# imalexlee/simple-vk-renderer

Hardware: AMD Instinct MI355X
Metric: shaded fragments/s (higher is better)
Workload: dtype f32

## Files before the change

simple-vk-renderer_amd/csrc/k_tile.hip:

```cpp
#include <hip/hip_ext.h>

#include <cstdlib>
#include <type_traits>

#include "svr_launch.h"
#include "svr_pixel.h"
#include "svr_span.h"

namespace svr {

constexpr uint32_t REC_COMMON = 0x80000000u;
#ifndef SVR_PRIO_COST
#define SVR_PRIO_COST 200u
#endif
constexpr int BATCH = 64;
constexpr uint32_t SREC = 7;

constexpr float kG0 = 0x1.c51282p-2f, kG1 = -0x1.14a3a2p-2f, kG2 = 0x1.37536ap-3f, kG3 = -0x1.778474p-5f;

__device__ __forceinline__ float lod_from_rho2(float rho2) {
  uint32_t bits = f2u(rho2);
  int e = (int)(bits >> 23) - 127;
  float m = u2f((bits & 0x7fffffu) | 0x3f800000u);
  float t = m - 1.0f;
  float g = fmaf(fmaf(fmaf(kG3, t, kG2), t, kG1), t, kG0);
  float s = t * (1.0f - t);
  float l = fmaf(s, g, t);
  float lam = 0.5f * ((float)e + l);
  lam = (rho2 <= 0x1p+100f) ? lam : 50.0f;
  lam = (rho2 >= 0x1p-100f) ? lam : -50.0f;
  return lam;
}

__device__ __forceinline__ float lerpf(float a, float b, float t) { return fmaf(t, b - a, a); }
__device__ __forceinline__ float clamp_med3(float x, float lo, float hi) { return __builtin_amdgcn_fmed3f(x, lo, hi); }
__device__ __forceinline__ double top_left_bias(uint32_t flags, uint32_t bit) { return (double)((flags / bit) & 1u); }

struct TexD {
  uint32_t base_off;
  uint32_t w, h, lw, lh, levels, filters;
  float min_lod, max_lod;
};

struct Taps {
  uint32_t o00, o10, o01, o11;
  float alpha, beta;
};
__device__ __forceinline__ Taps level_taps(int wl, int hl, uint32_t plw, uint32_t base, bool linear, float u, float v) {
  float U = (u - floorf(u)) * (float)wl;
  float V = (v - floorf(v)) * (float)hl;
  float Uh = U - 0.5f, Vh = V - 0.5f;
  float fu = floorf(linear ? Uh : U), fv = floorf(linear ? Vh : V);
  Taps tp;
  tp.alpha = linear ? Uh - fu : 0.0f;
  tp.beta = linear ? Vh - fv : 0.0f;
  int i0 = (int)fu, j0 = (int)fv;
  int i1 = linear ? i0 + 1 : i0, j1 = linear ? j0 + 1 : j0;
  if (i0 < 0) i0 += wl;
  if (i0 >= wl) i0 -= wl;
  if (i1 >= wl) i1 -= wl;
  if (j0 < 0) j0 += hl;
  if (j0 >= hl) j0 -= hl;
  if (j1 >= hl) j1 -= hl;
  const uint32_t x0 = texel_offset_x((uint32_t)i0), x1 = texel_offset_x((uint32_t)i1);
  const uint32_t y0 = base + texel_offset_y(plw, (uint32_t)j0), y1 = base + texel_offset_y(plw, (uint32_t)j1);
  tp.o00 = y0 + x0;
  tp.o10 = y0 + x1;
  tp.o01 = y1 + x0;
  tp.o11 = y1 + x1;
  return tp;
}
__device__ __forceinline__ Taps level_taps_exp(int kw, int kh, uint32_t plw, uint32_t base, float u, float v) {
  float U = ldexpf(u - floorf(u), kw);
  float V = ldexpf(v - floorf(v), kh);
  float Uh = U - 0.5f, Vh = V - 0.5f;
  float fu = floorf(Uh), fv = floorf(Vh);
  Taps tp;
  tp.alpha = Uh - fu;
  tp.beta = Vh - fv;
  const int i0 = (int)fu, j0 = (int)fv;
  const uint32_t mw = (1u << kw) - 1u, mh = (1u << kh) - 1u;
  const uint32_t x0 = texel_offset_x((uint32_t)i0 & mw), x1 = texel_offset_x((uint32_t)(i0 + 1) & mw);
  const uint32_t y0 = base + texel_offset_y(plw, (uint32_t)j0 & mh), y1 = base + texel_offset_y(plw, (uint32_t)(j0 + 1) & mh);
  tp.o00 = y0 + x0;
  tp.o10 = y0 + x1;
  tp.o01 = y1 + x0;
  tp.o11 = y1 + x1;
  return tp;
}
__device__ __forceinline__ uint32_t texel(const uint8_t* arena, uint32_t off) {
  return *reinterpret_cast<const uint32_t*>(arena + off);
}
__device__ __forceinline__ float bilerp(uint32_t t00, uint32_t t10, uint32_t t01, uint32_t t11, int c, float a, float b) {
  return lerpf(lerpf(chan(t00, c), chan(t10, c), a), lerpf(chan(t01, c), chan(t11, c), a), b);
}

__device__ __forceinline__ float4 common_texture(const uint8_t* tb, uint32_t base_off, uint32_t tk, uint32_t info, int dhi, int dlo,
                                                 float delta, float u, float v) {
  const uint32_t lw = info & 0xffu, lh = (info >> 8) & 0xffu;
  auto kexp = [](uint32_t l, int d) { return (int)__builtin_elementwise_sub_sat(l, (uint32_t)d); };
  const uint32_t bhi = base_off + packed_mip_offset(tk, (uint32_t)dhi);
  const Taps th = level_taps_exp(kexp(lw, dhi), kexp(lh, dhi), packed_level_lw(info, (uint32_t)dhi), bhi, u, v);
  const uint32_t h00 = texel(tb, th.o00), h10 = texel(tb, th.o10), h01 = texel(tb, th.o01), h11 = texel(tb, th.o11);
  float4 tx;
  tx.w = 1.0f;
  const bool two_levels = __any(delta != 0.0f);
  Taps tl = th;
  uint32_t l00 = 0, l10 = 0, l01 = 0, l11 = 0;
  if (two_levels) {
    const uint32_t blo = dlo != dhi ? bhi + packed_level_bytes(tk, (uint32_t)dhi) : bhi;
    tl = level_taps_exp(kexp(lw, dlo), kexp(lh, dlo), packed_level_lw(info, (uint32_t)dlo), blo, u, v);
    l00 = texel(tb, tl.o00), l10 = texel(tb, tl.o10), l01 = texel(tb, tl.o01), l11 = texel(tb, tl.o11);
  }
  tx.x = bilerp(h00, h10, h01, h11, 0, th.alpha, th.beta);
  tx.y = bilerp(h00, h10, h01, h11, 1, th.alpha, th.beta);
  tx.z = bilerp(h00, h10, h01, h11, 2, th.alpha, th.beta);
  if (two_levels) {
    tx.x = lerpf(tx.x, bilerp(l00, l10, l01, l11, 0, tl.alpha, tl.beta), delta);
    tx.y = lerpf(tx.y, bilerp(l00, l10, l01, l11, 1, tl.alpha, tl.beta), delta);
    tx.z = lerpf(tx.z, bilerp(l00, l10, l01, l11, 2, tl.alpha, tl.beta), delta);
  }
  return tx;
}

__device__ __forceinline__ float interp3(float a0, float da1, float da2, float b1, float b2, float r) {
  return fmaf(b2, da2, fmaf(b1, da1, a0)) * r;
}

struct FragAttr {
  float b1, b2, r, u, v, nx, ny, nz, light, cr, cg, cb, won;
};

__device__ __forceinline__ float quad_partner_x(float v) { return u2f((uint32_t)__builtin_amdgcn_mov_dpp((int)f2u(v), 0xB1, 0xf, 0xf, true)); }
__device__ __forceinline__ float quad_partner_y(float v) { return u2f((uint32_t)__builtin_amdgcn_mov_dpp((int)f2u(v), 0x128, 0xf, 0xf, true)); }
template <bool TRACE, bool COMMON = false, bool ATTR = false>
__device__ __forceinline__ float4 shade_pixel(const FrameParams& P, uint32_t rec, int px, int py, float* trace, const bool quads = false,
                                              FragAttr* fa = nullptr) {
  const TriRec* tr = P.recs + rec;
  const uint4* q4 = reinterpret_cast<const uint4*>(tr);
  const float4* f4 = reinterpret_cast<const float4*>(tr);
  const double2* d2 = reinterpret_cast<const double2*>(tr);
  uint4 hdr = q4[0];
  float4 zrow = f4[1];
  double2 c2 = d2[2], c3 = d2[3], c4 = d2[4], c5 = d2[5], c6 = d2[6];
  uint4 td = q4[7];
  float4 s0 = f4[8], s1 = f4[9], s2 = f4[10], s3 = f4[11], s4 = f4[12], s5 = f4[13], s6 = f4[14];
  uint32_t flags = hdr.w;
  float inv_area = zrow.w;
  double A1, B1, A2, B2, e1, e2;
  double C1 = c5.y, C2 = c6.x;
  A1 = c2.y; B1 = c4.x; A2 = c3.x; B2 = c4.y;
  double dx = (double)px, dy = (double)py;
  e1 = fma(A1, dx, fma(B1, dy, C1)) + top_left_bias(flags, F_T1);
  e2 = fma(A2, dx, fma(B2, dy, C2)) + top_left_bias(flags, F_T2);
  TexD t;
  t.base_off = (uint32_t)(unsigned long long)__double_as_longlong(c6.y);
  const uint32_t tk = (uint32_t)((unsigned long long)__double_as_longlong(c6.y) >> 32);
  t.w = td.x & 0xffffu;
  t.h = td.x >> 16;
  t.lw = td.y & 0xffu;
  t.lh = (td.y >> 8) & 0xffu;
  t.levels = (td.y >> 16) & 0xffu;
  t.filters = td.y >> 24;
  t.min_lod = u2f(td.z);
  t.max_lod = u2f(td.w);
  float b1 = (float)e1 * inv_area, b2 = (float)e2 * inv_area;
  float q0 = s0.x, dq1 = s0.y, dq2 = s0.z;
  const float qq = fmaf(b2, dq2, fmaf(b1, dq1, q0));
  float hb1 = 0.0f, hb2 = 0.0f, vb1 = 0.0f, vb2 = 0.0f, hq = 1.0f, vq = 1.0f, hr = 0.0f, vr = 0.0f;
  auto partners = [&]() {
    if (COMMON) {
      const int sx = (int)((uint32_t)px << 31), sy = (int)((uint32_t)py << 31);
      auto flip = [](double a, int s) { return __hiloint2double(__double2hiint(a) ^ s, __double2loint(a)); };
      hb1 = (float)(e1 + flip(A1, sx)) * inv_area, hb2 = (float)(e2 + flip(A2, sx)) * inv_area;
      vb1 = (float)(e1 + flip(B1, sy)) * inv_area, vb2 = (float)(e2 + flip(B2, sy)) * inv_area;
    } else {
      double sxp = (px & 1) ? -1.0 : 1.0, syp = (py & 1) ? -1.0 : 1.0;
      hb1 = (float)fma(sxp, A1, e1) * inv_area, hb2 = (float)fma(sxp, A2, e2) * inv_area;
      vb1 = (float)fma(syp, B1, e1) * inv_area, vb2 = (float)fma(syp, B2, e2) * inv_area;
    }
    hq = fmaf(hb2, dq2, fmaf(hb1, dq1, q0)), vq = fmaf(vb2, dq2, fmaf(vb1, dq1, q0));
  };
  if (!COMMON && !quads) partners();
  const float r = COMMON ? rcp_in_window(qq) : rcp_ieee(qq);
  const uint32_t kind = COMMON ? (uint32_t)PIPE_MESH : ((flags >> F_KIND_SHIFT) & 3u);
  float cr = interp3(s1.z, s3.z, s5.z, b1, b2, r);
  float cg = interp3(s1.w, s3.w, s5.w, b1, b2, r);
  float cb = interp3(s2.x, s4.x, s6.x, b1, b2, r);
  if (ATTR) { fa->b1 = b1; fa->b2 = b2; fa->r = r; fa->won = 1.0f; }
  if (kind == PIPE_COLORED_TRIANGLE) return make_float4(cr, cg, cb, 1.0f);
  float u = interp3(s2.y, s4.y, s6.y, b1, b2, r), v = interp3(s2.z, s4.z, s6.z, b1, b2, r);
  if (ATTR) { fa->u = u; fa->v = v; }
  if (!COMMON) {
    hr = rcp_ieee(hq);
    vr = rcp_ieee(vq);
  }
  float uh, vh, uv_, vv_;
  if (quads) {
    uh = quad_partner_x(u), vh = quad_partner_x(v);
    uv_ = quad_partner_y(u), vv_ = quad_partner_y(v);
  } else {
    if (COMMON) {
      partners();
      hr = rcp_in_window(hq);
      vr = rcp_in_window(vq);
    }
    uh = interp3(s2.y, s4.y, s6.y, hb1, hb2, hr), vh = interp3(s2.z, s4.z, s6.z, hb1, hb2, hr);
    uv_ = interp3(s2.y, s4.y, s6.y, vb1, vb2, vr), vv_ = interp3(s2.z, s4.z, s6.z, vb1, vb2, vr);
  }
  float dudx = (COMMON || !(px & 1)) ? (uh - u) : (u - uh);
  float dvdx = (COMMON || !(px & 1)) ? (vh - v) : (v - vh);
  float dudy = (COMMON || !(py & 1)) ? (uv_ - u) : (u - uv_);
  float dvdy = (COMMON || !(py & 1)) ? (vv_ - v) : (v - vv_);
  float W0 = (float)t.w, H0 = (float)t.h;
  float mx = COMMON ? ldexpf(dudx, (int)t.lw) : dudx * W0, my = COMMON ? ldexpf(dvdx, (int)t.lh) : dvdx * H0;
  float nx_ = COMMON ? ldexpf(dudy, (int)t.lw) : dudy * W0, ny_ = COMMON ? ldexpf(dvdy, (int)t.lh) : dvdy * H0;
  float rho2 = fmaxf(fmaf(mx, mx, my * my), fmaf(nx_, nx_, ny_ * ny_));
  float lambda = COMMON ? clamp_med3(lod_from_rho2(rho2), t.min_lod, t.max_lod) : fminf(fmaxf(lod_from_rho2(rho2), t.min_lod), t.max_lod);
  const bool linear = COMMON ? true : (((lambda <= 0.0f) ? (t.filters & 1u) : ((t.filters >> 1) & 1u)) != 0u);
  int q = COMMON ? (int)(tk >> 24) : (int)t.levels - 1;
  const bool mip_linear = COMMON ? true : (((t.filters >> 2) & 1u) != 0u);
  int dn = min(max((int)ceilf(lambda + 0.5f) - 1, 0), q);
  float lc = COMMON ? clamp_med3(lambda, 0.0f, (float)q) : fminf(fmaxf(lambda, 0.0f), (float)q);
  float fl = floorf(lc);
  int dhi = mip_linear ? (int)fl : dn;
  float delta = mip_linear ? lc - fl : 0.0f;
  int dlo = mip_linear ? min(dhi + 1, q) : dn;
  float us = (COMMON || fabsf(u) < 8388608.0f) ? u : 0.0f, vs = (COMMON || fabsf(v) < 8388608.0f) ? v : 0.0f;
  float4 tx;
  if constexpr (COMMON) {
    tx = common_texture(P.tex_arena, t.base_off, tk, td.y, dhi, dlo, delta, us, vs);
  } else {
    const int whi = (int)max(t.w >> dhi, 1u), hhi = (int)max(t.h >> dhi, 1u);
    const uint32_t bhi = t.base_off + mip_offset(t.lw, t.lh, (uint32_t)dhi);
    const uint32_t plw_hi = level_lw(t.lw, (uint32_t)dhi);
    Taps th = level_taps(whi, hhi, plw_hi, bhi, linear, us, vs);
    const uint8_t* tb = P.tex_arena;
    uint32_t h00 = texel(tb, th.o00), h10 = texel(tb, th.o10), h01 = texel(tb, th.o01), h11 = texel(tb, th.o11);
    const bool two_levels = __any(delta != 0.0f);
    Taps tl = th;
    uint32_t l00 = 0, l10 = 0, l01 = 0, l11 = 0;
    if (two_levels) {
      const int wlo = (int)max(t.w >> dlo, 1u), hlo = (int)max(t.h >> dlo, 1u);
      const uint32_t step = level_bytes(t.lw, t.lh, (uint32_t)dhi);
      const uint32_t blo = dlo != dhi ? bhi + step : bhi;
      const uint32_t plw_lo = level_lw(t.lw, (uint32_t)dlo);
      tl = level_taps(wlo, hlo, plw_lo, blo, linear, us, vs);
      l00 = texel(tb, tl.o00);
      l10 = texel(tb, tl.o10);
      l01 = texel(tb, tl.o01);
      l11 = texel(tb, tl.o11);
    }
    tx.x = bilerp(h00, h10, h01, h11, 0, th.alpha, th.beta);
    tx.y = bilerp(h00, h10, h01, h11, 1, th.alpha, th.beta);
    tx.z = bilerp(h00, h10, h01, h11, 2, th.alpha, th.beta);
    tx.w = 1.0f;
    if (two_levels) {
      tx.x = lerpf(tx.x, bilerp(l00, l10, l01, l11, 0, tl.alpha, tl.beta), delta);
      tx.y = lerpf(tx.y, bilerp(l00, l10, l01, l11, 1, tl.alpha, tl.beta), delta);
      tx.z = lerpf(tx.z, bilerp(l00, l10, l01, l11, 2, tl.alpha, tl.beta), delta);
    }
    if (TRACE) {
      trace[0] = (float)(hdr.z >> 2); trace[1] = b1; trace[2] = b2; trace[3] = r; trace[4] = u; trace[5] = v;
      trace[6] = dudx; trace[7] = dvdx; trace[8] = dudy; trace[9] = dvdy; trace[10] = lambda;
      trace[11] = tx.x; trace[12] = tx.y; trace[13] = tx.z;
      trace[26] = hb1; trace[27] = hb2; trace[28] = vb1; trace[29] = vb2; trace[30] = hr; trace[31] = vr;
    }
    if (kind == PIPE_TEX_IMAGE) {
      tx.w = bilerp(h00, h10, h01, h11, 3, th.alpha, th.beta);
      if (two_levels) tx.w = lerpf(tx.w, bilerp(l00, l10, l01, l11, 3, tl.alpha, tl.beta), delta);
      return tx;
    }
  }
  float nx = interp3(s0.w, s2.w, s4.w, b1, b2, r);
  float ny = interp3(s1.x, s3.x, s5.x, b1, b2, r);
  float nz = interp3(s1.y, s3.y, s5.y, b1, b2, r);
  const float* L = P.scene.sunlight_direction;
  float d = fmaf(nz, L[2], fmaf(ny, L[1], nx * L[0]));
  float light = fmaxf(d, 0.1f);
  float sunw = P.scene.sunlight_color[3];
  cr = cr * tx.x;
  cg = cg * tx.y;
  cb = cb * tx.z;
  float4 o;
  o.x = fmaf(cr * light, sunw, cr * P.scene.ambient_color[0]);
  o.y = fmaf(cg * light, sunw, cg * P.scene.ambient_color[1]);
  o.z = fmaf(cb * light, sunw, cb * P.scene.ambient_color[2]);
  o.w = 1.0f;
  if (TRACE) {
    trace[15] = nx; trace[16] = ny; trace[17] = nz; trace[18] = cr; trace[19] = cg; trace[20] = cb;
    trace[21] = light; trace[22] = o.x; trace[23] = o.y; trace[24] = o.z; trace[25] = o.w;
  }
  if (ATTR) { fa->nx = nx; fa->ny = ny; fa->nz = nz; fa->light = light; fa->cr = cr; fa->cg = cg; fa->cb = cb; }
  return o;
}

template <bool INSTR, bool LIST, bool HIZ>
__device__ __forceinline__ void scan_columns(const FrameParams& P, uint4* s_cov, const uint32_t* s_list, uint32_t bin_base, uint32_t n,
                                             unsigned long long* s_depth, uint32_t* s_bm, int tx0, int ty0, int ry0, int nrows,
                                             uint32_t& n_raster, uint32_t& n_hiz_bad, uint32_t& occl) {
  auto entry = [&](uint32_t i) -> uint32_t { return LIST ? (s_list[i] & 0x7fffffffu) : P.bins[bin_base + i]; };
  const uint32_t lane = threadIdx.x & 63u, wave = threadIdx.x >> 6;
  static_assert(BATCH * 8 == 512, "two pieces per thread");
  uint4 pre0 = make_uint4(0, 0, 0, 0), pre1 = pre0;
  {
    uint32_t cnt = min((uint32_t)BATCH, n);
    const bool staged = (threadIdx.x & 7u) < SREC;
    if (staged && threadIdx.x < cnt * 8u) pre0 = reinterpret_cast<const uint4*>(P.recs + entry(threadIdx.x >> 3))[threadIdx.x & 7u];
    if (staged && threadIdx.x + 256u < cnt * 8u) pre1 = reinterpret_cast<const uint4*>(P.recs + entry(32u + (threadIdx.x >> 3)))[threadIdx.x & 7u];
  }
  constexpr uint32_t SVR_HIZ_MIN = BATCH;
  constexpr uint32_t SVR_HIZ_KEEP_COLS = 192u;
  const bool hiz = HIZ && n > (uint32_t)SVR_HIZ_MIN;
  uint32_t cur = 0, hz_cols = 0, hz_batches = 0, hz_pause = 0;
  if (hiz && threadIdx.x < 32u) s_bm[threadIdx.x] = threadIdx.x < 16u ? 0u : 0xffffffffu;
  for (uint32_t b0 = 0; b0 < n; b0 += BATCH) {
    uint32_t cnt = min((uint32_t)BATCH, n - b0);
    __syncthreads();
    const bool test = hiz && b0 && hz_pause == 0u;
    if (hiz && b0 && hz_pause) hz_pause--;
    if (test) {
      cur ^= 1u;
      const uint32_t b = threadIdx.x >> 4, k = threadIdx.x & 15u;
      const uint4* c4 = reinterpret_cast<const uint4*>(s_depth + ((b & 3u) * 8u + (k >> 1)) * TILE + (b >> 2) * 8u + (k & 1u) * 4u);
      const uint4 lo = c4[0], hi = c4[1];
      atomicMin(&s_bm[cur * 16u + b], min(min(lo.y, lo.w), min(hi.y, hi.w)));
      if (threadIdx.x < 16u) s_bm[(cur ^ 1u) * 16u + threadIdx.x] = 0xffffffffu;
    }
    if (threadIdx.x < cnt * 8u && (threadIdx.x & 7u) < SREC) s_cov[(threadIdx.x >> 3) * SREC + (threadIdx.x & 7u)] = pre0;
    if (threadIdx.x + 256u < cnt * 8u && (threadIdx.x & 7u) < SREC) s_cov[(32u + (threadIdx.x >> 3)) * SREC + (threadIdx.x & 7u)] = pre1;
    __syncthreads();
    const uint4* bm4 = reinterpret_cast<const uint4*>(s_bm + cur * 16u);
    if (b0 + BATCH < n) {
      uint32_t nb = b0 + BATCH, ncnt = min((uint32_t)BATCH, n - nb);
      const bool staged = (threadIdx.x & 7u) < SREC;
      if (staged && threadIdx.x < ncnt * 8u) pre0 = reinterpret_cast<const uint4*>(P.recs + entry(nb + (threadIdx.x >> 3)))[threadIdx.x & 7u];
      if (staged && threadIdx.x + 256u < ncnt * 8u) pre1 = reinterpret_cast<const uint4*>(P.recs + entry(nb + 32u + (threadIdx.x >> 3)))[threadIdx.x & 7u];
    }
    int cx0 = 0, cw = 0;
    bool hidden = false;
    uint32_t gone = 0;
    uint32_t zb = 0, claim = 0;
    if (lane < cnt) {
      uint4 h = s_cov[lane * SREC];
      int minx = (int)(int16_t)(h.x & 0xffffu), miny = (int)(int16_t)(h.x >> 16);
      int maxx = (int)(int16_t)(h.y & 0xffffu), maxy = (int)(int16_t)(h.y >> 16);
      cx0 = max(minx, tx0);
      const int cx1 = min(maxx, tx0 + TILE - 1);
      const int cy0 = max(miny, ry0), cy1 = min(maxy, ry0 + nrows - 1);
      cw = (cx1 >= cx0 && cy1 >= cy0) ? cx1 - cx0 + 1 : 0;
      if (HIZ && cw) {
        const float4 zr = reinterpret_cast<const float4*>(s_cov)[lane * SREC + 1u];
        const float eps = (fabsf(zr.x) + fabsf(zr.y) + fabsf(zr.z)) * 0x1p-21f;
        zb = f2u(fmaxf(fmaxf(zr.x, fmaxf(zr.x + zr.y, zr.x + zr.z)) + eps, 0.0f));
        if (minx <= tx0 && maxx >= tx0 + TILE - 1 && miny <= ry0 && maxy >= ry0 + nrows - 1) {
          const double* dd = reinterpret_cast<const double*>(s_cov + lane * SREC);
          const float x0 = (float)tx0, x1 = (float)(tx0 + TILE - 1), y0 = (float)ry0, y1 = (float)(ry0 + nrows - 1);
          bool all_in = true;
          float slack = 0.0f;
          float bc[2][4];
#pragma unroll
          for (int i = 0; i < 3; i++) {
            const float A = (float)dd[4 + i], B = (float)dd[7 + i], C = (float)dd[10 + i] + ((i == 1 && (h.w & F_T1)) || (i == 2 && (h.w & F_T2)) ? 1.0f : 0.0f);
            const float M = (fabsf(C) + fmaxf(fabsf(A * x0), fabsf(A * x1)) + fmaxf(fabsf(B * y0), fabsf(B * y1))) * 0x1p-21f;
            const float e00 = fmaf(A, x0, fmaf(B, y0, C)), e10 = fmaf(A, x1, fmaf(B, y0, C));
            const float e01 = fmaf(A, x0, fmaf(B, y1, C)), e11 = fmaf(A, x1, fmaf(B, y1, C));
            all_in = all_in && fminf(fminf(e00, e10), fminf(e01, e11)) >= M + 1.0f;
            if (i) {
              bc[i - 1][0] = e00 * zr.w; bc[i - 1][1] = e10 * zr.w; bc[i - 1][2] = e01 * zr.w; bc[i - 1][3] = e11 * zr.w;
              slack = fmaxf(slack, M * zr.w);
            }
          }
          if (all_in) {
            float zmin = fmaf(bc[1][0], zr.z, fmaf(bc[0][0], zr.y, zr.x));
            zmin = fminf(zmin, fmaf(bc[1][1], zr.z, fmaf(bc[0][1], zr.y, zr.x)));
            zmin = fminf(zmin, fmaf(bc[1][2], zr.z, fmaf(bc[0][2], zr.y, zr.x)));
            zmin = fminf(zmin, fmaf(bc[1][3], zr.z, fmaf(bc[0][3], zr.y, zr.x)));
            zmin -= eps + 2.0f * slack * (fabsf(zr.y) + fabsf(zr.z));
            claim = f2u(fminf(fmaxf(zmin, 0.0f), 1.0f));
          }
        }
      }
    }
    if (HIZ) {
      unsigned long long claims = __ballot(claim != 0u);
      while (claims) {
        const int l = __ffsll((long long)claims) - 1;
        claims &= claims - 1ull;
        occl = max(occl, (uint32_t)__builtin_amdgcn_readlane((int)claim, l));
      }
      if (!INSTR && cw && zb < occl) cw = 0;
    }
    if (lane < cnt) {
      if (test && cw) {
        const uint4 h = s_cov[lane * SREC];
        const int cx1 = min((int)(int16_t)(h.y & 0xffffu), tx0 + TILE - 1);
        const int cy0 = max((int)(int16_t)(h.x >> 16), ry0), cy1 = min((int)(int16_t)(h.y >> 16), ry0 + nrows - 1);
        uint32_t m = 0xffffffffu;
        const int by0 = (cy0 - ty0) >> 3, by1 = (cy1 - ty0) >> 3;
        for (int bx = (cx0 - tx0) >> 3; bx <= (cx1 - tx0) >> 3; bx++) {
          const uint4 q = bm4[bx];
          m = min(m, (by0 <= 0 && by1 >= 0) ? q.x : 0xffffffffu);
          m = min(m, (by0 <= 1 && by1 >= 1) ? q.y : 0xffffffffu);
          m = min(m, (by0 <= 2 && by1 >= 2) ? q.z : 0xffffffffu);
          m = min(m, (by0 <= 3 && by1 >= 3) ? q.w : 0xffffffffu);
        }
        hidden = zb < m;
        if (hidden) gone = (uint32_t)cw;
        if (!INSTR && hidden) cw = 0;
      }
      if (INSTR && cw) {
        uint32_t* fl = reinterpret_cast<uint32_t*>(s_cov) + lane * SREC * 4u + 3u;
        *fl = (*fl & 0x7fffffffu) | ((hidden || (LIST && (s_list[b0 + lane] >> 31))) ? 0x80000000u : 0u);
      }
    }
    if (test) {
      const uint32_t nh = (uint32_t)__popcll(__ballot(hidden));
      hz_cols += nh + 3u * (uint32_t)__popcll(__ballot(gone >= 4u)) + 12u * (uint32_t)__popcll(__ballot(gone >= 16u));
      if (++hz_batches == 2u) {
        if (hz_cols < SVR_HIZ_KEEP_COLS) hz_pause = 6u;
        hz_cols = hz_batches = 0u;
      }
    }
    uint32_t inc = (uint32_t)cw;
#pragma unroll
    for (int off = 1; off < 64; off <<= 1) {
      uint32_t v = __shfl_up(inc, off);
      if ((int)lane >= off) inc += v;
    }
    uint32_t total = (uint32_t)__builtin_amdgcn_readlane((int)inc, 63);
    const uint32_t sh = total <= 64u ? 2u : (total <= 128u ? 1u : 0u);
    const int band_rows = nrows >> sh;
    const uint32_t items = total << sh;
    for (uint32_t c = wave; c * 64u < items; c += 4u) {
      uint32_t item = c * 64u + lane;
      uint32_t j = item >> sh, band = item & ((1u << sh) - 1u);
      bool act = item < items;
      uint32_t pos = 0;
#pragma unroll
      for (uint32_t step = 32; step >= 1; step >>= 1) {
        uint32_t v = __shfl(inc, (int)min(pos + step - 1u, 63u));
        if (pos + step <= 64u && v <= j) pos += step;
      }
      uint32_t i = min(pos, 63u);
      uint32_t excl = __shfl(inc, (int)i) - (uint32_t)__shfl(cw, (int)i);
      int col = __shfl(cx0, (int)i) + (int)(j - excl);
      if (!act) continue;
      const uint4* rec = s_cov + i * SREC;
      uint4 h = rec[0];
      int miny = (int)(int16_t)(h.x >> 16), maxy = (int)(int16_t)(h.y >> 16);
      int y0 = max(miny, ry0 + (int)band * band_rows), y1 = min(maxy, ry0 + (int)band * band_rows + band_rows - 1);
      if (y0 > y1) continue;
      uint32_t key = h.z, flags = h.w;
      float4 zr = reinterpret_cast<const float4*>(rec)[1];
      const double2* d = reinterpret_cast<const double2*>(rec);
      double2 c2 = d[2], c3 = d[3], c4 = d[4], c5 = d[5], c6 = d[6];
      double B0 = c3.y, B1 = c4.x, B2 = c4.y;
      double u1 = top_left_bias(flags, F_T1), u2 = top_left_bias(flags, F_T2);
      double dx = (double)col, dy = (double)y0;
      double f0 = fma(c2.x, dx, fma(B0, dy, c5.x));
      double f1 = fma(c2.y, dx, fma(B1, dy, c5.y));
      double f2 = fma(c3.x, dx, fma(B2, dy, c6.x));
      int k0, kn;
      svr_span::column_span(f0, f1, f2, B0, B1, B2, y1 - y0 + 1, k0, kn);
      if (kn == 0) continue;
      if (INSTR) n_raster += (uint32_t)kn;
      const double dk = (double)k0;
      double g1 = fma(B1, dk, f1) + u1, g2 = fma(B2, dk, f2) + u2;
      unsigned long long* cell = s_depth + (y0 + k0 - ty0) * TILE + (col - tx0);
      for (; kn > 0; kn--) {
        float b1 = (float)g1 * zr.w, b2 = (float)g2 * zr.w;
        float z = fmaf(b2, zr.z, fmaf(b1, zr.y, zr.x));
        z = fminf(fmaxf(z, 0.0f), 1.0f) + 0.0f;
        if (INSTR && (flags >> 31) && f2u(z) >= (uint32_t)(*cell >> 32)) n_hiz_bad++;
        atomicMax(cell, ((unsigned long long)f2u(z) << 32) | key);
        g1 += B1;
        g2 += B2;
        cell += TILE;
      }
    }
  }
}

__device__ __forceinline__ uint32_t resolve_record(const FrameParams& P, uint32_t rec, int px, int py) {
  uint4 h = *reinterpret_cast<const uint4*>(P.recs + rec);
  if ((int)(int16_t)(h.x & 0xffffu) <= (int)(int16_t)(h.y & 0xffffu)) return rec;
  double dx = (double)px, dy = (double)py;
  for (uint32_t c = 0; c < h.w; c++) {
    const TriRec* t = P.recs + h.z + c;
    if (t->minx > t->maxx || px < t->minx || px > t->maxx || py < t->miny || py > t->maxy) continue;
    if (fma(t->A[0], dx, fma(t->B[0], dy, t->C[0])) >= 0.0 && fma(t->A[1], dx, fma(t->B[1], dy, t->C[1])) >= 0.0 &&
        fma(t->A[2], dx, fma(t->B[2], dy, t->C[2])) >= 0.0)
      return h.z + c;
  }
  return rec;
}

constexpr uint32_t SORT_CAP = SPLIT_SORT_MAX;
constexpr uint32_t RANK_SORT_MAX = 1024;
#ifndef SVR_HIZ_FILTER_MIN
#define SVR_HIZ_FILTER_MIN 1024
#endif
constexpr uint32_t HIZ_AVG_ENTRIES = 96;
constexpr uint32_t HIZ_FILTER_MIN = SVR_HIZ_FILTER_MIN;
constexpr uint32_t QUARTER_LIST_CAP = 3808;
constexpr uint32_t QUEUE_CAP = 128;

template <int FMT, bool INSTR>
__device__ __forceinline__ void flush_fragments(const FrameParams& P, typename Codec<FMT>::enc_t* col, uint2* q,
                                                float4* s_src, uint32_t& qn, int tx0, int by0,
                                                uint32_t lane, uint32_t& n_shaded) {
  typedef Codec<FMT> CD;
  uint32_t cnt = min(qn, 64u);
  bool act = lane < cnt;
  uint2 e = q[act ? lane : 0u];
  uint32_t pix = e.x, rec = e.y;
  int px = tx0 + (int)(pix & 31u), py = by0 + (int)(pix >> 5);
  float4 src = make_float4(0.f, 0.f, 0.f, 0.f);
  if (__all(!act || (rec & REC_COMMON))) {
    if (act) src = shade_pixel<false, true>(P, rec & ~REC_COMMON, px, py, nullptr);
  } else if (act) {
    src = shade_pixel<false>(P, rec & ~REC_COMMON, px, py, nullptr);
  }
  if (INSTR && act) n_shaded++;
  if (act) s_src[lane] = src;
  unsigned long long mm = __ballot(act);
#pragma unroll
  for (uint32_t b = 0; b < 8u; b++) {
    const bool bit = (pix >> b) & 1u;
    const unsigned long long with = __ballot(bit);
    mm &= bit ? with : ~with;
  }
  mm = act ? mm : 0ull;
  __builtin_amdgcn_wave_barrier();
  if (act && (mm & ((1ull << lane) - 1ull)) == 0ull) {
    float4 dst = CD::decode(col[pix]);
    typename CD::enc_t out = col[pix];
    while (mm) {
      uint32_t j = (uint32_t)__ffsll((long long)mm) - 1u;
      mm &= mm - 1ull;
      float4 sj = s_src[j];
      float4 o = make_float4(fmaf(dst.x, dst.w, sj.x), fmaf(dst.y, dst.w, sj.y), fmaf(dst.z, dst.w, sj.z), sj.w);
      if (INSTR && P.trace_buf && px == P.trace_x && py == P.trace_y) {
        (void)shade_pixel<true>(P, q[j].y & ~REC_COMMON, px, py, P.trace_buf);
        float* tb = P.trace_buf;
        tb[32] = dst.x; tb[33] = dst.y; tb[34] = dst.z; tb[35] = dst.w;
        tb[36] = o.x; tb[37] = o.y; tb[38] = o.z; tb[39] = o.w;
      }
      out = CD::encode(o);
      dst = CD::decode(out);
    }
    col[pix] = out;
  }
  uint32_t rest = qn - cnt;
  for (uint32_t j = lane; j < rest; j += 64u) {
    uint2 v = q[cnt + j];
    q[j] = v;
  }
  qn = rest;
}

__device__ __forceinline__ uint32_t tid_of(uint32_t wv) {
  uint32_t lane;
  asm volatile("v_mbcnt_lo_u32_b32 %0, -1, 0\n\tv_mbcnt_hi_u32_b32 %0, -1, %0" : "=v"(lane));
  return (wv << 6) | lane;
}

template <int SLOT>
__device__ __forceinline__ bool block_any(bool v, uint32_t wv) {
  __shared__ __attribute__((aligned(16))) uint32_t votes[2][4];
  votes[SLOT][wv] = __any(v) ? 1u : 0u;
  __syncthreads();
  const uint4 all = *reinterpret_cast<const uint4*>(votes[SLOT]);
  return (all.x | all.y | all.z | all.w) != 0u;
}

template <int FMT, bool INSTR>
__device__ __forceinline__ void scan_columns_ordered(const FrameParams& P, uint4* s_cov, uint32_t* s_idx, const uint32_t* order,
                                                     uint32_t n, int tx0, int ty0, int row0, uint32_t lrpw, const uint32_t* s_z,
                                                     typename Codec<FMT>::enc_t* col, uint2* q, float4* s_src,
                                                     uint32_t& n_raster, uint32_t& n_shaded, const uint32_t wv) {
  const uint32_t tid = tid_of(wv), lane = tid & 63u, wave = wv;
  const unsigned long long below = (1ull << lane) - 1ull;
  const int rpw = 1 << lrpw;
  const int by0 = ty0 + row0 + rpw * (int)wave, by1 = by0 + rpw - 1;
  uint32_t qn = 0;
  for (uint32_t b0 = 0; b0 < n; b0 += BATCH) {
    uint32_t cnt = min((uint32_t)BATCH, n - b0);
    __syncthreads();
    {
      const uint32_t st = tid_of(wv), t0 = st >> 3, pc = st & 7u;
      uint32_t ri0 = 0, ri1 = 0;
      if (t0 < cnt) ri0 = order[b0 + t0];
      if (t0 + 32u < cnt) ri1 = order[b0 + 32u + t0];
      uint4 r0 = make_uint4(0, 0, 0, 0), r1 = r0;
      if (t0 < cnt && pc < SREC) r0 = reinterpret_cast<const uint4*>(P.recs + ri0)[pc];
      if (t0 + 32u < cnt && pc < SREC) r1 = reinterpret_cast<const uint4*>(P.recs + ri1)[pc];
      if (t0 < cnt) {
        if (pc < SREC) s_cov[t0 * SREC + pc] = r0;
        if (pc == 0) s_idx[t0] = ri0;
      }
      if (t0 + 32u < cnt) {
        if (pc < SREC) s_cov[(t0 + 32u) * SREC + pc] = r1;
        if (pc == 0) s_idx[t0 + 32u] = ri1;
      }
    }
    __syncthreads();
    int cx0 = 0, cw = 0;
    if (lane < cnt) {
      uint4 h = s_cov[lane * SREC];
      int minx = (int)(int16_t)(h.x & 0xffffu), miny = (int)(int16_t)(h.x >> 16);
      int maxx = (int)(int16_t)(h.y & 0xffffu), maxy = (int)(int16_t)(h.y >> 16);
      cx0 = max(minx, tx0);
      int cx1 = min(maxx, tx0 + TILE - 1);
      cw = (cx1 >= cx0 && min(maxy, by1) >= max(miny, by0)) ? cx1 - cx0 + 1 : 0;
    }
    uint32_t inc = (uint32_t)cw;
#pragma unroll
    for (int off = 1; off < 64; off <<= 1) {
      uint32_t v = __shfl_up(inc, off);
      if ((int)lane >= off) inc += v;
    }
    uint32_t total = (uint32_t)__builtin_amdgcn_readlane((int)inc, 63);
    uint32_t c = 0;
    int t = 0;
    for (;;) {
      bool full = false;
      while (c * 64u < total) {
        uint32_t j = c * 64u + lane;
        bool act = j < total;
        uint32_t pos = 0;
#pragma unroll
        for (uint32_t step = 32; step >= 1; step >>= 1) {
          uint32_t v = __shfl(inc, (int)min(pos + step - 1u, 63u));
          if (pos + step <= 64u && v <= j) pos += step;
        }
        uint32_t i = min(pos, 63u);
        uint32_t excl = __shfl(inc, (int)i) - (uint32_t)__shfl(cw, (int)i);
        int colx = __shfl(cx0, (int)i) + (int)(j - excl) - tx0;
        colx = act ? colx : 0;
        const uint4* rec = s_cov + i * SREC;
        uint4 h = rec[0];
        int y0 = (int)(int16_t)(h.x >> 16), y1 = (int)(int16_t)(h.y >> 16);
        uint32_t flags = h.w, ri = s_idx[i];
        float4 zr = reinterpret_cast<const float4*>(rec)[1];
        const double2* d = reinterpret_cast<const double2*>(rec);
        double2 c2 = d[2], c3 = d[3], c4 = d[4], c5 = d[5], c6 = d[6];
        double B0 = c3.y, B1 = c4.x, B2 = c4.y;
        double dx = (double)(tx0 + colx), dy = (double)(by0 + t);
        double f0 = fma(c2.x, dx, fma(B0, dy, c5.x));
        const double u1 = top_left_bias(flags, F_T1), u2 = top_left_bias(flags, F_T2);
        double g1 = fma(c2.y, dx, fma(B1, dy, c5.y));
        double g2 = fma(c3.x, dx, fma(B2, dy, c6.x));
#pragma unroll 1
        for (; t < rpw; t++) {
          int y = by0 + t;
          bool inside = act && y >= y0 && y <= y1 && f0 >= 0.0 && g1 >= 0.0 && g2 >= 0.0;
          if (INSTR) n_raster += inside ? 1u : 0u;
          float b1 = (float)(g1 + u1) * zr.w, b2 = (float)(g2 + u2) * zr.w;
          float z = fmaf(b2, zr.z, fmaf(b1, zr.y, zr.x));
          z = fminf(fmaxf(z, 0.0f), 1.0f) + 0.0f;
          bool pass = inside && f2u(z) >= s_z[(y - ty0) * TILE + colx];
          unsigned long long m = __ballot(pass);
          f0 += B0;
          g1 += B1;
          g2 += B2;
          if (m) {
            if (pass) q[qn + (uint32_t)__popcll(m & below)] = make_uint2((uint32_t)(t * TILE + colx), ri | ((h.z & 2u) ? REC_COMMON : 0u));
            qn += (uint32_t)__popcll(m);
            if (qn >= 64u) {
              full = true;
              t++;
              break;
            }
          }
        }
        if (full) break;
        t = 0;
        c++;
      }
      if (!full) break;
      flush_fragments<FMT, INSTR>(P, col, q, s_src, qn, tx0, by0, lane, n_shaded);
      if (t == rpw) {
        t = 0;
        c++;
      }
    }
  }
  while (qn) flush_fragments<FMT, INSTR>(P, col, q, s_src, qn, tx0, by0, lane, n_shaded);
}

template <uint32_t K, typename KeyT>
__device__ __forceinline__ void count_ranks(const KeyT* s, uint32_t n, const KeyT (&mine)[K], uint32_t (&rank)[K]) {
#pragma unroll
  for (uint32_t k = 0; k < K; k++) rank[k] = 0;
  for (uint32_t j = 0; j < n; j++) {
    KeyT v = s[j];
#pragma unroll
    for (uint32_t k = 0; k < K; k++) rank[k] += v < mine[k] ? 1u : 0u;
  }
}

template <uint32_t K>
__device__ __forceinline__ void rank_sort(const FrameParams& P, unsigned char* lds, uint32_t bin_base, uint32_t n, uint32_t* out, const uint32_t wv) {
  const uint32_t tid = tid_of(wv);
  uint32_t* k32 = reinterpret_cast<uint32_t*>(lds);
  uint32_t* claim = k32 + SORT_CAP;
  uint32_t ri[K], key[K], rank[K];
#pragma unroll
  for (uint32_t k = 0; k < K; k++) {
    uint32_t i = tid + 256u * k;
    ri[k] = i < n ? P.bins[bin_base + i] : 0u;
  }
#pragma unroll
  for (uint32_t k = 0; k < K; k++) {
    uint32_t i = tid + 256u * k;
    key[k] = i < n ? P.recs[ri[k]].key : 0u;
    if (i < n) k32[i] = key[k];
  }
  __syncthreads();
  count_ranks<K, uint32_t>(k32, n, key, rank);
#pragma unroll
  for (uint32_t k = 0; k < K; k++) {
    uint32_t i = tid + 256u * k;
    if (i < n) claim[rank[k]] = i;
  }
  __syncthreads();
  bool lost = false;
#pragma unroll
  for (uint32_t k = 0; k < K; k++) {
    uint32_t i = tid + 256u * k;
    lost = lost || (i < n && claim[rank[k]] != i);
  }
  if (block_any<0>(lost, wv)) {
    unsigned long long* k64 = reinterpret_cast<unsigned long long*>(lds);
    unsigned long long wide[K];
#pragma unroll
    for (uint32_t k = 0; k < K; k++) {
      uint32_t i = tid + 256u * k;
      wide[k] = ((unsigned long long)key[k] << 32) | ri[k];
      if (i < n) k64[i] = wide[k];
    }
    __syncthreads();
    count_ranks<K, unsigned long long>(k64, n, wide, rank);
  }
#pragma unroll
  for (uint32_t k = 0; k < K; k++)
    if (tid + 256u * k < n) out[rank[k]] = ri[k];
}

template <uint32_t K>
__device__ __forceinline__ void rank_pass(const uint32_t* k32, const uint32_t* r32, uint32_t* marks, uint32_t base, uint32_t n, uint32_t* out, const uint32_t wv) {
  const uint32_t tid = tid_of(wv);
  uint32_t mine[K], rank[K];
#pragma unroll
  for (uint32_t k = 0; k < K; k++) {
    uint32_t i = base + tid + 256u * k;
    mine[k] = i < n ? k32[i] : 0xffffffffu;
  }
  count_ranks<K, uint32_t>(k32, n, mine, rank);
#pragma unroll
  for (uint32_t k = 0; k < K; k++) {
    uint32_t i = base + tid + 256u * k;
    if (i < n) {
      out[rank[k]] = r32[i];
      marks[rank[k]] = 1u;
    }
  }
}

__device__ __forceinline__ void rank_sort_big(const FrameParams& P, unsigned char* lds, uint32_t* marks, uint32_t bin_base, uint32_t n,
                                              uint32_t* out, const uint32_t wv) {
  const uint32_t tid = tid_of(wv);
  uint32_t* k32 = reinterpret_cast<uint32_t*>(lds);
  uint32_t* r32 = k32 + SORT_CAP;
  {
    uint32_t ri[8], key[8];
#pragma unroll
    for (uint32_t k = 0; k < 8; k++) {
      uint32_t i = tid + 256u * k;
      ri[k] = i < n ? P.bins[bin_base + i] : 0u;
    }
#pragma unroll
    for (uint32_t k = 0; k < 8; k++) {
      uint32_t i = tid + 256u * k;
      key[k] = i < n ? P.recs[ri[k]].key : 0u;
    }
#pragma unroll
    for (uint32_t k = 0; k < 8; k++) {
      uint32_t i = tid + 256u * k;
      if (i < n) {
        k32[i] = key[k];
// ... 844 lines not shown
```

simple-vk-renderer_amd/csrc/svr_device.h:

```cpp
#pragma once

#include <hip/hip_runtime.h>
#include <stdint.h>

#include "../../include/svr.h"

namespace svr {

constexpr int TILE = 32;
constexpr int TILE_SHIFT = 5;
constexpr int WAVE = 64;
constexpr float GUARD = 16384.0f;
constexpr uint32_t NO_REC = 0xffffffffu;
#ifndef SVR_RCP_VARIANT
#define SVR_RCP_VARIANT 1
#endif

enum PipelineKind : uint32_t { PIPE_MESH = 0, PIPE_COLORED_TRIANGLE = 1, PIPE_TEX_IMAGE = 2 };

constexpr uint32_t F_T1 = 1u;
constexpr uint32_t F_T2 = 2u;
constexpr uint32_t F_KIND_SHIFT = 4;
constexpr uint32_t F_TRANSPARENT = 256u;
constexpr uint32_t F_VIEW_SHIFT = 24;
// ... 147 lines not shown
static_assert(sizeof(TriRec) == 256, "TriRec layout");
static_assert(offsetof(TriRec, object) == 240, "TriRec layout: the ID words are piece 15's x and y");
constexpr uint32_t REC_ID_PIECE = offsetof(TriRec, object) / 16u;
static_assert(offsetof(TriRec, A) == 32 && offsetof(TriRec, tex_off) == 104 && offsetof(TriRec, tex_wh) == 112 &&
                  offsetof(TriRec, q0) == 128, "TriRec layout");

struct ClipItem {
  uint32_t draw;
  uint32_t tri;
};

struct Counters {
  uint32_t n_clip;
  uint32_t n_extra;
  uint32_t total_entries;
  uint32_t overflow;
  unsigned long long rasterized;
  unsigned long long shaded;
  unsigned long long binned;
  uint32_t n_big;
  uint32_t n_pairs;
  uint32_t n_pairs_rest;
  uint32_t sort_used;
  uint32_t n_split;
  uint32_t cost_sum;
  uint32_t flat_draws;
  uint32_t flat_tris;
  uint32_t flat_chunks;
  uint32_t flat_culled;
  uint32_t hiz_bad;
  uint32_t occl_tested;
  uint32_t occl_culled;
  uint32_t occl_tris;
};
static_assert(sizeof(Counters) == 96, "Counters layout");

struct MeshEntry {
  const SvrVertex* vtx;
  const uint32_t* idx;
  const float* groups;
  uint64_t pad;
};
struct MatEntry {
  float cf[4];
  uint32_t pass;
  uint32_t pad[3];
};

constexpr uint32_t PYR_MAX_LEVELS = 14;

struct FrameParams {
  void* color;
  float* depth;
  uint32_t W, H;
  uint32_t sx, sy, sw, sh;
  uint32_t tiles_x, tiles_y, n_tiles;
  uint32_t rstride, roff;
  uint32_t depth_load;
  const DrawDesc* draws;
  const WaveChunk* chunks;
  uint32_t n_chunks;
  uint32_t n_tris;
  TriRec* recs;
  uint32_t extra_cap;
  ClipItem* clip_queue;
  uint32_t clip_cap;
  uint32_t* big_queue;
  uint32_t* tile_count;
  uint32_t* tile_offset;
  uint32_t* cls_count;
  uint32_t* row_cost;
  uint32_t* host_row_cost;
  Counters* host_counters;
  uint32_t* host_failed_seq;
  uint32_t op_seq;
  uint32_t lazy_clear;
  uint32_t clear_lo, clear_hi;
  uint32_t flatten;
  uint32_t* poison;
  uint2* pairs;
  uint32_t* pair_slot;
  uint4* tile_info;
  unsigned long long* sort_arena;
  uint32_t sort_cap;
  uint32_t* tile_order;
  uint32_t* bins;
  uint32_t bin_cap;
  Counters* counters;
  const TexBinding* tex;
  const uint8_t* tex_arena;
  uint32_t instrument;
  int trace_x, trace_y;
  float* trace_buf;
  uint32_t* tile_cycles;
  uint32_t tuning;
  uint32_t layer_rows;
  SvrSceneData scene;
  uint2* ids;
  const uint32_t* pyr;
  uint32_t pyr_levels;
  uint32_t pyr_off[PYR_MAX_LEVELS + 1];
  uint8_t* occl_flags;
  void* attr[4];
  unsigned long long* host_clock;
};
constexpr uint32_t CLOCK_STRIDE = 16;
constexpr uint32_t CLOCK_WORDS = 65 * CLOCK_STRIDE;

constexpr uint32_t LIST_FUSED_MAX = 4096;

struct FlattenParams {
  const SvrRenderObject* objects;
  SvrRenderObject* objects_dev;
  uint32_t n_opaque, n_transparent;
  float viewproj[16];
  const MeshEntry* meshes;
  const MatEntry* materials;
  unsigned long long* keys;
  uint32_t* draw_tris;
  uint32_t* chunk_base;
  DrawDesc* draws;
  WaveChunk* chunks;
  Counters* counters;
  uint32_t ids;
  const uint32_t* obj_ids;
  uint32_t n_views;
  const float* viewprojs;
};

__device__ __forceinline__ int tile_row_y(const FrameParams& P, int ty) {
  return (int)P.sy + (ty * (int)P.rstride + (int)P.roff) * TILE;
}
__device__ __forceinline__ void local_tile_rows(const FrameParams& P, int miny, int maxy, int& l0, int& l1) {
  const int g0 = (miny - (int)P.sy) >> TILE_SHIFT, g1 = (maxy - (int)P.sy) >> TILE_SHIFT;
  l0 = g0;
  l1 = g1;
  if (P.rstride > 1u) {
    const int s = (int)P.rstride, b = g1 - (int)P.roff;
    l0 = (g0 - (int)P.roff + s - 1) / s;
    l1 = b < 0 ? -1 : b / s;
  }
}

template <bool MV>
__device__ __forceinline__ uint32_t bin_base(const FrameParams& P, uint32_t flags) {
  uint32_t b = (flags & F_TRANSPARENT) ? P.n_tiles : 0u;
  if (MV) b += (flags >> F_VIEW_SHIFT) * P.layer_rows * P.tiles_x;
  return b;
}

__device__ __forceinline__ float u2f(uint32_t u) { return __uint_as_float(u); }
__device__ __forceinline__ uint32_t f2u(float f) { return __float_as_uint(f); }

template <int VARIANT>
__device__ __forceinline__ float rcp_refined(float x) {
  float y = __builtin_amdgcn_rcpf(x);
  float r = fmaf(-x, y, 1.0f);
  y = fmaf(r, y, y);
  if (VARIANT == 2) {
    r = fmaf(-x, y, 1.0f);
    y = fmaf(r, y, y);
  }
  return y;
}
__device__ __forceinline__ bool rcp_fast_ok(float x) {
  return ((f2u(x) >> 23) & 0xffu) - 32u <= 190u;
}
__device__ __forceinline__ float rcp_ieee(float x) {
#ifdef SVR_AB_PLAIN_DIV
  return 1.0f / x;
#endif
  if (__builtin_expect(!rcp_fast_ok(x), 0)) return 1.0f / x;
  return rcp_refined<SVR_RCP_VARIANT>(x);
}
__device__ __forceinline__ float rcp_in_window(float x) {
#ifdef SVR_AB_PLAIN_DIV
  return 1.0f / x;
#else
  return rcp_refined<SVR_RCP_VARIANT>(x);
#endif
}

struct VOut {
  float clip[4];
  float attr[8];
};

__device__ __forceinline__ void matvec4(const float* m, float x, float y, float z, float w, float* out) {
#pragma unroll
  for (int r = 0; r < 4; r++) {
    float acc = m[0 + r] * x;
    acc = fmaf(m[4 + r], y, acc);
    acc = fmaf(m[8 + r], z, acc);
    acc = fmaf(m[12 + r], w, acc);
    out[r] = acc;
  }
}
struct Vec4 {
  float x, y, z, w;
};
__device__ __forceinline__ Vec4 mat_vec(const float* m, float x, float y, float z, float w) {
  Vec4 r;
  r.x = m[0] * x; r.y = m[1] * x; r.z = m[2] * x; r.w = m[3] * x;
  r.x = fmaf(m[4], y, r.x); r.y = fmaf(m[5], y, r.y); r.z = fmaf(m[6], y, r.z); r.w = fmaf(m[7], y, r.w);
  r.x = fmaf(m[8], z, r.x); r.y = fmaf(m[9], z, r.y); r.z = fmaf(m[10], z, r.z); r.w = fmaf(m[11], z, r.w);
  r.x = fmaf(m[12], w, r.x); r.y = fmaf(m[13], w, r.y); r.z = fmaf(m[14], w, r.z); r.w = fmaf(m[15], w, r.w);
  return r;
}
__device__ __forceinline__ void matmul4(const float* a, const float* b, float* out) {
#pragma unroll
  for (int j = 0; j < 4; j++) matvec4(a, b[4 * j + 0], b[4 * j + 1], b[4 * j + 2], b[4 * j + 3], out + 4 * j);
}

struct VertexRaw {
  float4 a, b, c;
};
__device__ __forceinline__ VertexRaw load_vertex(const SvrVertex* base, uint32_t index) {
  const float4* p = reinterpret_cast<const float4*>(base + index);
  VertexRaw v;
  v.a = p[0];
  v.b = p[1];
  v.c = p[2];
  return v;
}

__device__ __forceinline__ void mesh_vert(const VertexRaw& v, const float* mvp, const float* world,
                                          const float* color_factors, VOut& o) {
  matvec4(mvp, v.a.x, v.a.y, v.a.z, 1.0f, o.clip);
#pragma unroll
  for (int r = 0; r < 3; r++) {
    float acc = world[0 + r] * v.b.x;
    acc = fmaf(world[4 + r], v.b.y, acc);
    acc = fmaf(world[8 + r], v.b.z, acc);
    o.attr[r] = acc;
  }
  o.attr[3] = v.c.x * color_factors[0];
  o.attr[4] = v.c.y * color_factors[1];
  o.attr[5] = v.c.z * color_factors[2];
  o.attr[6] = v.a.w;
  o.attr[7] = v.b.w;
}

__device__ __forceinline__ void colored_triangle_mesh_vert(const VertexRaw& v, const float* render_matrix, VOut& o) {
  matvec4(render_matrix, v.a.x, v.a.y, v.a.z, 1.0f, o.clip);
  o.attr[0] = o.attr[1] = o.attr[2] = 0.0f;
  o.attr[3] = v.c.x;
  o.attr[4] = v.c.y;
  o.attr[5] = v.c.z;
  o.attr[6] = v.a.w;
  o.attr[7] = v.b.w;
}

__device__ __forceinline__ void colored_triangle_vert(int i, VOut& o) {
  o.clip[0] = (i == 0) ? 1.0f : (i == 1 ? -1.0f : 0.0f);
  o.clip[1] = (i == 2) ? -1.0f : 1.0f;
  o.clip[2] = 0.0f;
  o.clip[3] = 1.0f;
#pragma unroll
  for (int k = 0; k < 8; k++) o.attr[k] = 0.0f;
  o.attr[3] = (i == 0) ? 1.0f : 0.0f;
  o.attr[4] = (i == 1) ? 1.0f : 0.0f;
  o.attr[5] = (i == 2) ? 1.0f : 0.0f;
}

enum { OC_NEAR = 1, OC_FAR = 2, OC_L = 4, OC_R = 8, OC_T = 16, OC_B = 32 };
__device__ __forceinline__ int outcode(const float* c) {
  int oc = 0;
  if (c[2] > c[3]) oc |= OC_NEAR;
  if (c[2] < 0.0f) oc |= OC_FAR;
  if (c[0] < -c[3]) oc |= OC_L;
  if (c[0] > c[3]) oc |= OC_R;
  if (c[1] < -c[3]) oc |= OC_T;
  if (c[1] > c[3]) oc |= OC_B;
  return oc;
}

struct ScreenV {
  float xs, ys, zs, rw;
  bool ok;
};
__device__ __forceinline__ ScreenV to_screen(const float* c, float hw, float hh) {
  ScreenV s;
  s.rw = rcp_ieee(c[3]);
  s.xs = fmaf(c[0] * s.rw, hw, hw);
  s.ys = fmaf(c[1] * s.rw, hh, hh);
  s.zs = c[2] * s.rw;
  s.ok = (fabsf(s.xs) <= GUARD) && (fabsf(s.ys) <= GUARD);
  return s;
}

__device__ __forceinline__ void store_invalid(TriRec* rec) {
  uint4 h;
  h.x = 1u;
  h.y = 0u;
  h.z = 0u;
  h.w = 0u;
  *reinterpret_cast<uint4*>(rec) = h;
}

__device__ __forceinline__ uint32_t make_key(uint32_t seq, uint32_t draw_flags, const TexBinding& tex, bool clipped) {
  bool pow2 = (tex.wh & 0xffffu) == (1u << (tex.info & 0xffu)) && (tex.wh >> 16) == (1u << ((tex.info >> 8) & 0xffu));
  bool common = ((draw_flags >> F_KIND_SHIFT) & 3u) == PIPE_MESH && (tex.info >> 24) == 7u && pow2;
  return ((seq + 1u) << 2) | (common ? 2u : 0u) | (clipped ? 1u : 0u);
}

struct TriGeom {
// ... 108 lines not shown
```

Baseline: 49.64 billion.

## Replace per-item binary search with LDS tag scatter and DPP wave scans

Replaces the shuffle-based inclusive prefix sum with a DPP-based wave scan. It also replaces the per-item 6-step binary search over the prefix array, which maps a work item to its owning primitive and column, with a scatter-then-max-scan. Each primitive's starting item writes a packed owner/column tag into a per-wave LDS scratch area after the staged records. A max-scan then propagates each tag to the lanes that follow it, with a carry taken from the previous chunk. This cuts the many cross-lane shuffles per chunk, at the cost of LDS writes, wave barriers and reliance on the spare shared-memory space and the tag bit packing.

```diff
diff --git a/simple-vk-renderer_amd/csrc/k_tile.hip b/simple-vk-renderer_amd/csrc/k_tile.hip
--- a/simple-vk-renderer_amd/csrc/k_tile.hip
+++ b/simple-vk-renderer_amd/csrc/k_tile.hip
@@ -4,6 +4,7 @@
 #include <type_traits>
 
 #include "svr_launch.h"
+#include "svr_items.h"
 #include "svr_pixel.h"
 #include "svr_span.h"
 
@@ -295,12 +296,30 @@
   return o;
 }
 
+static_assert((BATCH * 8 - BATCH * SREC) * sizeof(uint4) >= 4 * svr_items::CHUNK * sizeof(uint32_t), "64 words per wave behind the staged records");
+__device__ __forceinline__ uint32_t* item_tag_words(uint4* s_cov, uint32_t wave) {
+  return reinterpret_cast<uint32_t*>(s_cov + BATCH * SREC) + wave * svr_items::CHUNK;
+}
+__device__ __forceinline__ uint32_t item_tags(uint32_t* words, uint32_t lane, uint32_t first, uint32_t tag, uint32_t c) {
+  const uint32_t pos = svr_items::chunk_pos(first, c);
+  words[lane] = 0u;
+  __builtin_amdgcn_wave_barrier();
+  if (pos < svr_items::CHUNK) words[pos] = tag;
+  __builtin_amdgcn_wave_barrier();
+  const uint32_t t = words[lane];
+  const unsigned long long before = __ballot(svr_items::begins_before(first, c));
+  uint32_t carry = 0u;
+  if (before) carry = (uint32_t)__builtin_amdgcn_readlane((int)tag, 63 - __clzll((long long)before));
+  return max(wave_scan_max(t), carry);
+}
+
 template <bool INSTR, bool LIST, bool HIZ>
 __device__ __forceinline__ void scan_columns(const FrameParams& P, uint4* s_cov, const uint32_t* s_list, uint32_t bin_base, uint32_t n,
                                              unsigned long long* s_depth, uint32_t* s_bm, int tx0, int ty0, int ry0, int nrows,
                                              uint32_t& n_raster, uint32_t& n_hiz_bad, uint32_t& occl) {
   auto entry = [&](uint32_t i) -> uint32_t { return LIST ? (s_list[i] & 0x7fffffffu) : P.bins[bin_base + i]; };
   const uint32_t lane = threadIdx.x & 63u, wave = threadIdx.x >> 6;
+  uint32_t* const tag_words = item_tag_words(s_cov, wave);
   static_assert(BATCH * 8 == 512, "two pieces per thread");
   uint4 pre0 = make_uint4(0, 0, 0, 0), pre1 = pre0;
   {
@@ -422,29 +441,20 @@
         hz_cols = hz_batches = 0u;
       }
     }
-    uint32_t inc = (uint32_t)cw;
-#pragma unroll
-    for (int off = 1; off < 64; off <<= 1) {
-      uint32_t v = __shfl_up(inc, off);
-      if ((int)lane >= off) inc += v;
-    }
+    const uint32_t inc = wave_scan_add((uint32_t)cw);
     uint32_t total = (uint32_t)__builtin_amdgcn_readlane((int)inc, 63);
-    const uint32_t sh = total <= 64u ? 2u : (total <= 128u ? 1u : 0u);
+    const uint32_t sh = svr_items::band_shift(total);
     const int band_rows = nrows >> sh;
     const uint32_t items = total << sh;
+    const uint32_t first = svr_items::first_item(inc - (uint32_t)cw, (uint32_t)cw, sh);
+    const uint32_t tag = svr_items::make_tag(lane, cx0 - tx0, inc - (uint32_t)cw);
     for (uint32_t c = wave; c * 64u < items; c += 4u) {
       uint32_t item = c * 64u + lane;
       uint32_t j = item >> sh, band = item & ((1u << sh) - 1u);
       bool act = item < items;
-      uint32_t pos = 0;
-#pragma unroll
-      for (uint32_t step = 32; step >= 1; step >>= 1) {
-        uint32_t v = __shfl(inc, (int)min(pos + step - 1u, 63u));
-        if (pos + step <= 64u && v <= j) pos += step;
-      }
-      uint32_t i = min(pos, 63u);
-      uint32_t excl = __shfl(inc, (int)i) - (uint32_t)__shfl(cw, (int)i);
-      int col = __shfl(cx0, (int)i) + (int)(j - excl);
+      const uint32_t t = item_tags(tag_words, lane, first, tag, c);
+      const uint32_t i = svr_items::tag_owner(t);
+      const int col = tx0 + svr_items::tag_column(t, j);
       if (!act) continue;
       const uint4* rec = s_cov + i * SREC;
       uint4 h = rec[0];
@@ -582,6 +592,7 @@
                                                      uint32_t& n_raster, uint32_t& n_shaded, const uint32_t wv) {
   const uint32_t tid = tid_of(wv), lane = tid & 63u, wave = wv;
   const unsigned long long below = (1ull << lane) - 1ull;
+  uint32_t* const tag_words = item_tag_words(s_cov, wave);
   const int rpw = 1 << lrpw;
   const int by0 = ty0 + row0 + rpw * (int)wave, by1 = by0 + rpw - 1;
   uint32_t qn = 0;
@@ -615,13 +626,10 @@
       int cx1 = min(maxx, tx0 + TILE - 1);
       cw = (cx1 >= cx0 && min(maxy, by1) >= max(miny, by0)) ? cx1 - cx0 + 1 : 0;
     }
-    uint32_t inc = (uint32_t)cw;
-#pragma unroll
-    for (int off = 1; off < 64; off <<= 1) {
-      uint32_t v = __shfl_up(inc, off);
-      if ((int)lane >= off) inc += v;
-    }
+    const uint32_t inc = wave_scan_add((uint32_t)cw);
     uint32_t total = (uint32_t)__builtin_amdgcn_readlane((int)inc, 63);
+    const uint32_t first = svr_items::first_item(inc - (uint32_t)cw, (uint32_t)cw, 0u);
+    const uint32_t tag = svr_items::make_tag(lane, cx0 - tx0, inc - (uint32_t)cw);
     uint32_t c = 0;
     int t = 0;
     for (;;) {
@@ -629,15 +637,9 @@
       while (c * 64u < total) {
         uint32_t j = c * 64u + lane;
         bool act = j < total;
-        uint32_t pos = 0;
-#pragma unroll
-        for (uint32_t step = 32; step >= 1; step >>= 1) {
-          uint32_t v = __shfl(inc, (int)min(pos + step - 1u, 63u));
-          if (pos + step <= 64u && v <= j) pos += step;
-        }
-        uint32_t i = min(pos, 63u);
-        uint32_t excl = __shfl(inc, (int)i) - (uint32_t)__shfl(cw, (int)i);
-        int colx = __shfl(cx0, (int)i) + (int)(j - excl) - tx0;
+        const uint32_t tg = item_tags(tag_words, lane, first, tag, c);
+        const uint32_t i = svr_items::tag_owner(tg);
+        int colx = svr_items::tag_column(tg, j);
         colx = act ? colx : 0;
         const uint4* rec = s_cov + i * SREC;
         uint4 h = rec[0];
diff --git a/simple-vk-renderer_amd/csrc/svr_device.h b/simple-vk-renderer_amd/csrc/svr_device.h
--- a/simple-vk-renderer_amd/csrc/svr_device.h
+++ b/simple-vk-renderer_amd/csrc/svr_device.h
@@ -323,6 +323,27 @@
 __device__ __forceinline__ float u2f(uint32_t u) { return __uint_as_float(u); }
 __device__ __forceinline__ uint32_t f2u(float f) { return __float_as_uint(f); }
 
+#define SVR_WAVE_SCAN(OP)                                                                                          \
+  v = OP(v, (uint32_t)__builtin_amdgcn_update_dpp(0, (int)v, 0x111, 0xf, 0xf, false));              \
+  v = OP(v, (uint32_t)__builtin_amdgcn_update_dpp(0, (int)v, 0x112, 0xf, 0xf, false));              \
+  v = OP(v, (uint32_t)__builtin_amdgcn_update_dpp(0, (int)v, 0x114, 0xf, 0xf, false));              \
+  v = OP(v, (uint32_t)__builtin_amdgcn_update_dpp(0, (int)v, 0x118, 0xf, 0xf, false));              \
+  v = OP(v, (uint32_t)__builtin_amdgcn_update_dpp(0, (int)v, 0x142, 0xa, 0xf, false));           \
+  v = OP(v, (uint32_t)__builtin_amdgcn_update_dpp(0, (int)v, 0x143, 0xc, 0xf, false));
+#define SVR_SCAN_ADD(a, b) ((a) + (b))
+#define SVR_SCAN_MAX(a, b) max((a), (b))
+__device__ __forceinline__ uint32_t wave_scan_add(uint32_t v) {
+  SVR_WAVE_SCAN(SVR_SCAN_ADD)
+  return v;
+}
+__device__ __forceinline__ uint32_t wave_scan_max(uint32_t v) {
+  SVR_WAVE_SCAN(SVR_SCAN_MAX)
+  return v;
+}
+#undef SVR_SCAN_ADD
+#undef SVR_SCAN_MAX
+#undef SVR_WAVE_SCAN
+
 template <int VARIANT>
 __device__ __forceinline__ float rcp_refined(float x) {
   float y = __builtin_amdgcn_rcpf(x);
diff --git a/simple-vk-renderer_amd/csrc/svr_items.h b/simple-vk-renderer_amd/csrc/svr_items.h
--- /dev/null
+++ b/simple-vk-renderer_amd/csrc/svr_items.h
@@ -0,0 +1,29 @@
+#pragma once
+
+#include <stdint.h>
+
+namespace svr_items {
+
+constexpr uint32_t CHUNK = 64;
+constexpr uint32_t TAG_SHIFT = 12;
+constexpr uint32_t TAG_LOW = (1u << TAG_SHIFT) - 1u;
+constexpr int TAG_BIAS = 2016;
+constexpr uint32_t NO_ITEM = 0xffffffffu;
+
+__host__ __device__ inline uint32_t band_shift(uint32_t total) { return total <= 64u ? 2u : (total <= 128u ? 1u : 0u); }
+
+__host__ __device__ inline uint32_t first_item(uint32_t excl, uint32_t cw, uint32_t sh) { return cw ? excl << sh : NO_ITEM; }
+
+__host__ __device__ inline uint32_t chunk_pos(uint32_t first, uint32_t c) { return first - c * CHUNK; }
+
+__host__ __device__ inline bool begins_before(uint32_t first, uint32_t c) { return first < c * CHUNK; }
+
+__host__ __device__ inline uint32_t make_tag(uint32_t lane, int cx0_rel, uint32_t excl) {
+  return (lane << TAG_SHIFT) | (uint32_t)(cx0_rel - (int)excl + TAG_BIAS);
+}
+
+__host__ __device__ inline uint32_t tag_owner(uint32_t tag) { return tag >> TAG_SHIFT; }
+
+__host__ __device__ inline int tag_column(uint32_t tag, uint32_t j) { return (int)(tag & TAG_LOW) - TAG_BIAS + (int)j; }
+
+}
```

Result: no change. 49.78 billion, median of 2 (+0.3%).
